# int-brain-lab/mtscomp

Hardware: AMD Instinct MI355X
Metric: compress + decompress GB/s (raw int16) (higher is better)
Workload: dtype int16

## Files before the change

### mtscomp_amd/csrc/inflate.hip

```cpp
#include <stdlib.h>

#include <vector>

#include "common.h"

namespace mts {

struct BitIn {
    const u32 *w;
    u64 nwords;
    u64 widx;
    u64 buf;
    u32 cnt;
    u32 nextw;
    u64 pos;
    u64 end;
    const u32 *lw = nullptr;
    u64 lw0 = 0;
    u32 lwn = 0;
    __device__ __forceinline__ void init(const u8 *base, u64 byte_off, u64 byte_len, u64 start_bit)
    {
        const u64 a = (u64)(base + byte_off);
        w = (const u32 *)(a & ~(u64)3);
        const u64 bit0 = (a & 3) * 8;
// ... 675 lines not shown
            if (o2 < 12) t0 |= (u64)k << (5 * o2); else t1 |= (u64)k << (5 * (o2 - 12));
        }
    }
    s.t0 = t0; s.t1 = t1;
    s.nlen = nlen; s.total = nlen + ndist;
    s.idx = 0; s.prev = 0; s.len256 = 0; s.maxl = 0; s.maxd = 0; s.kl = 0; s.kd = 0;
    return true;
}

__device__ __forceinline__ int vh_step(VhState &s)
{
    BitIn &br = s.br;
    br.refill();
    const u32 pk = br.peek();
    const u32 v7 = __brev(pk) >> 25, vb = __builtin_amdgcn_perm(v7, v7, 0u) | 0x80808080u;
    const u32 nge = (u32)__popc((vb - s.lima) & 0x80808080u) + (u32)__popc((vb - s.limb) & 0x80808080u);
    const u32 clen = 1 + nge;
    const int si = (int)(((u32)(s.so64 >> (8 * nge)) & 0xffu) + ((v7 - ((u32)(s.lo64 >> (8 * nge)) & 0xffu)) >> (6 - nge)));
    const int sym = (int)((si < 12 ? s.t0 >> (5 * si) : s.t1 >> (5 * (si - 12))) & 31);
    const u32 t4 = 4u * (u32)(max(sym, 15) - 15);
    const u32 xb = (0x7320u >> t4) & 15u;
    const int rep = (int)(((0xb331u >> t4) & 15u) + __builtin_amdgcn_ubfe(pk, clen, xb));
    br.skip(clen + xb);
    const int idx = s.idx, nlen = s.nlen;
    const int val = sym < 16 ? sym : sym == 16 ? s.prev : 0;
    if (sym >= 16 && ((sym == 16 && idx == 0) || idx + rep > s.total)) return -1;
    s.prev = val;
    if (val) {
        const int nl = idx >= nlen ? 0 : (idx + rep <= nlen ? rep : nlen - idx);
        const int nd = rep - nl;
        s.kl += (u32)nl << (15 - val);
        s.kd += (u32)nd << (15 - val);
        if (nl && val > s.maxl) s.maxl = val;
        if (nd && val > s.maxd) s.maxd = val;
        if (idx <= 256 && 256 < idx + rep) s.len256 = val;
        if (s.kl > 32768u || s.kd > 32768u) return -1;
    }
    s.idx = idx + rep;
    if (br.pos > br.end) return -1;
    if (s.idx < s.total) return 0;
    if (s.len256 == 0) return -1;
    if (s.kl > 32768u || (s.kl < 32768u && s.maxl != 1)) return -1;
    if (s.kd > 32768u || (s.kd < 32768u && s.maxd > 1)) return -1;
    return 1;
}

struct InfFast {
    u64 cand_off;
    u32 cand_cap;
    u32 true_off;
    u32 true_cap;
    u32 pad;
};
struct CandRes {
    u64 end_bit;
    u32 ntok, nout, nsub;
    u32 ok;
    u32 bfinal;
    u32 rows;
};
struct TrueBlk {
    u64 start_bit;
    u32 cand;
    u32 tok_off;
    u32 ntok;
    u32 chunk;
};
constexpr int PASSA_STAGE_WORDS = 64 * 1024 / 32 + 16;
#ifndef MTS_PASSB_STAGE_WORDS
#define MTS_PASSB_STAGE_WORDS 2304
#endif
constexpr int PASSB_STAGE_WORDS = MTS_PASSB_STAGE_WORDS;
constexpr int SUBCAP = 512;
constexpr u32 SUB_BITS = 1024;
#ifndef MTS_SUB_TARGET
#define MTS_SUB_TARGET 1024
#endif
constexpr u32 SUB_TARGET = MTS_SUB_TARGET;
constexpr u32 SUB_MIN = 256;
#ifndef MTS_INF_ROWCAP
#define MTS_INF_ROWCAP 192
#endif
constexpr u32 ROWCAP = MTS_INF_ROWCAP;
constexpr int ROUNDS_MAX = (SUBCAP + 63) / 64;
static inline u64 rows_rounds_of(u64 c_len) { return c_len * 8 / (64 * 640) + 32; }

#ifndef MTS_SCAN_SPANS
#define MTS_SCAN_SPANS 1
#endif
#ifndef MTS_PA_LEAN
#define MTS_PA_LEAN 1
#endif
constexpr int SCAN_SPANS = MTS_SCAN_SPANS;
constexpr u64 SCAN_FINAL_ZONE_BITS = 8ull * 256 * 1024;
constexpr int SCAN_L1_CAP = 14336;

__global__ __launch_bounds__(SCAN_THREADS) void k_inf_scan(const u8 *__restrict__ cdata, const InfChunk *__restrict__ chunks,
                                                           const InfFast *__restrict__ fast, u64 *__restrict__ cand_pos,
                                                           u32 *__restrict__ cand_cnt, u64 *__restrict__ surv_list,
                                                           u32 *__restrict__ surv_cnt, u32 surv_cap, u64 final_zone_bits)
{
    const int ci = blockIdx.y;
    const InfChunk ch = chunks[ci];
    if (ch.c_len < 8) return;
    const u64 a = (u64)(cdata + ch.c_off);
    const u32 *w = (const u32 *)(a & ~(u64)3);
    const u64 bit0 = (a & 3) * 8, end = bit0 + 8 * ch.c_len, nwords = (end + 31) >> 5;
    if ((u64)blockIdx.x * SCAN_SPANS * SCAN_SPAN_BITS >= end) return;
    __shared__ u32 sw[SCAN_THREADS + SCAN_TAIL];
    __shared__ u16 l1[SCAN_L1_CAP];
    __shared__ u32 surv[SCAN_SURV_CAP];
    __shared__ u32 wsum[16];
    __shared__ u32 nsurv;
    __shared__ u8 ktab[4096];
    const int tid = threadIdx.x, wave = tid >> 6, lane = tid & 63;
    for (int i = tid; i < 4096; i += SCAN_THREADS) {
        u32 k = 0;
        for (int f = 0; f < 4; f++) k += (0x80u >> ((i >> (3 * f)) & 7)) & 0x7f;
        ktab[i] = (u8)(k < 255 ? k : 255);
    }
    __shared__ u32 gbase_s;
    for (int sp = 0; sp < SCAN_SPANS; sp++) {
    const u64 span0 = ((u64)blockIdx.x * SCAN_SPANS + sp) * SCAN_SPAN_BITS;
    if (span0 >= end) break;
    const u64 word0 = span0 >> 5;
    __syncthreads();
    for (int i = tid; i < SCAN_THREADS + SCAN_TAIL; i += SCAN_THREADS) sw[i] = word0 + i < nwords ? w[word0 + i] : 0;
    if (tid == 0) nsurv = 0;
    __syncthreads();
    const u32 w0 = sw[tid], w1 = sw[tid + 1];
#define S_(j) __builtin_amdgcn_alignbit(w1, w0, j)
    u32 m = ~S_(1) & S_(2);
    m &= ~(S_(4) & S_(5) & S_(6) & S_(7));
    m &= ~(S_(9) & S_(10) & S_(11) & S_(12));
#undef S_
    if (span0 + SCAN_SPAN_BITS + final_zone_bits <= end) m &= ~w0;
    {
        const u64 o0 = span0 + (u64)tid * 32;
        const u64 first_ok = bit0 + 16;
        if (o0 + 32 <= first_ok || o0 + 100 > end) {
            u32 keep = 0;
            for (int k = 0; k < 32; k++) if (o0 + k >= first_ok && o0 + k + 100 <= end) keep |= 1u << k;
            m &= keep;
        } else if (o0 < first_ok) m &= ~0u << (u32)(first_ok - o0);
    }
    const u32 cntm = __popc(m);
    const u32 incl = wave_incl_scan_dpp(cntm), ex = incl - cntm;
    if (lane == 63) wsum[wave] = incl;
    __syncthreads();
    u32 base = 0, n1 = 0;
    for (int q = 0; q < 16; q++) { if (q < wave) base += wsum[q]; n1 += wsum[q]; }
    n1 = n1 < (u32)SCAN_L1_CAP ? n1 : (u32)SCAN_L1_CAP;
    {
        u32 slot = base + ex, mm = m;
        while (mm) {
            const int k = __ffs(mm) - 1;
            mm &= mm - 1;
            if (slot < (u32)SCAN_L1_CAP) l1[slot] = (u16)(tid * 32 + k);
            slot++;
        }
    }
    __syncthreads();
    for (u32 it = tid; it < n1; it += SCAN_THREADS) {
        const u32 rel = l1[it];
        const u32 wi = rel >> 5, k = rel & 31;
        const u32 x0 = sw[wi], x1 = sw[wi + 1], x2 = sw[wi + 2], x3 = sw[wi + 3];
// ... 71 lines not shown
                    }
                    active = vh_setup(s, w, nwords, end, o, row, VAL_STAGE);
                }
            }
            if (!__any(active)) {
                if (base + cnt >= stop) break;
                continue;
            }
        }
        for (int k = 0; k < VAL_STEPS; k++) {
            if (active) {
                const int r = vh_step(s);
                if (r) {
                    active = false;
                    if (r > 0) {
                        const InfFast f = fast[ci];
                        const u32 slot = atomicAdd(&cand_cnt[ci], 1u);
                        if (slot < f.cand_cap) cand_pos[f.cand_off + slot] = o;
                    }
                }
            }
        }
    }
}

__global__ __launch_bounds__(256) void k_inf_sortc(const InfFast *__restrict__ fast, u64 *__restrict__ cand_pos,
                                                   u64 *__restrict__ cand_tmp, u32 *__restrict__ cand_cnt)
{
    const int ci = blockIdx.x;
    const InfFast f = fast[ci];
    const u32 n = min(cand_cnt[ci], f.cand_cap);
    u64 *p = cand_pos + f.cand_off, *t = cand_tmp + f.cand_off;
    for (u32 i = threadIdx.x; i < n; i += 256) t[i] = p[i];
    __syncthreads();
    for (u32 i = threadIdx.x; i < n; i += 256) {
        const u64 v = t[i];
        u32 r = 0;
        for (u32 j = 0; j < n; j++) r += t[j] < v;
        p[r] = v;
    }
}

enum { SPAN_CONT = 0, SPAN_EOB = 1, SPAN_ERR = 2 };

template <int MODE>
__device__ __forceinline__ void decode_span(BitIn &br, LaneLds &L, const u32 *lutl, const u32 *lutd, u64 stop, u32 &ntok, u32 &nout,
                                            int &flag, u32 *tk, u32 want)
{
    flag = SPAN_CONT;
    ntok = 0; nout = 0;
    for (;;) {
        if (MODE == 2) { if (ntok >= want) break; }
        else if (br.pos >= stop) break;
        u32 tok, olen;
        const int t = decode_token_lut(br, L, lutl, lutd, tok, olen);
        if (t < 0 || br.pos > br.end) { flag = SPAN_ERR; break; }
        if (t == 1) { flag = SPAN_EOB; break; }
        const u32 np = lz_pieces(tok, olen);
        if (MODE == 2) lz_emit_pieces(tk + ntok, tok, olen);
        ntok += np; nout += olen;
    }
}

template <int MODE>
__device__ __forceinline__ void decode_span_fast(BitL &br, LaneLds &L, const u32 *lutl, const u32 *lutd, u32 stop, u32 end, u32 &ntok,
                                                 u32 &nout, int &flag, u32 *tk, u32 want)
{
    flag = SPAN_CONT;
    ntok = 0; nout = 0;
    for (;;) {
        if (MODE == 2) { if (ntok >= want) break; }
        else if (br.pos >= stop) break;
        u32 tok, olen;
        const int t = decode_token_lut(br, L, lutl, lutd, tok, olen);
        if (t < 0 || br.pos > end) { flag = SPAN_ERR; break; }
        if (t == 1) { flag = SPAN_EOB; break; }
        const u32 np = lz_pieces(tok, olen);
        if (MODE == 2) lz_emit_pieces(tk + ntok, tok, olen);
        ntok += np; nout += olen;
    }
}

__device__ __forceinline__ void decode_span_rows(BitL &br, LaneLds &L, const u32 *lutl, const u32 *lutd, u32 stop, u32 end, u32 &ntok,
                                                 u32 &nout, int &flag, u32 *row, u32 cap, bool &ovf)
{
    flag = SPAN_CONT;
    ntok = 0; nout = 0; ovf = false;
    for (;;) {
        if (br.pos >= stop) break;
        u32 tok, olen;
        const int t = decode_token_lut(br, L, lutl, lutd, tok, olen);
        if (t < 0 || br.pos > end) { flag = SPAN_ERR; break; }
        if (t == 1) { flag = SPAN_EOB; break; }
        const u32 np = lz_pieces(tok, olen);
        if (ntok + np <= cap) lz_emit_pieces(row + ntok, tok, olen);
        else ovf = true;
        ntok += np; nout += olen;
    }
}

__device__ __forceinline__ void decode_span_exit_w(BitW &br, LaneLds &L, const u32 *lutl, const u32 *lutd, u32 stop, u32 end, int &flag)
{
    flag = SPAN_CONT;
    for (;;) {
        if (br.pos >= stop) break;
        u32 tok, olen;
        const int t = decode_token_w(br, L, lutl, lutd, tok, olen);
        if (t < 0 || br.pos > end) { flag = SPAN_ERR; break; }
        if (t == 1) { flag = SPAN_EOB; break; }
    }
}
__device__ __forceinline__ void decode_span_rows_w(BitW &br, LaneLds &L, const u32 *lutl, const u32 *lutd, u32 stop, u32 end, u32 &ntok,
                                                   u32 &nout, int &flag, u32 *row, u32 cap, bool &ovf)
{
    flag = SPAN_CONT;
    ntok = 0; nout = 0; ovf = false;
    for (;;) {
        if (br.pos >= stop) break;
        u32 tok, olen;
        const int t = decode_token_w(br, L, lutl, lutd, tok, olen);
        if (t < 0 || br.pos > end) { flag = SPAN_ERR; break; }
        if (t == 1) { flag = SPAN_EOB; break; }
        const u32 np = lz_pieces(tok, olen);
        if (ntok + np <= cap) lz_emit_pieces(row + ntok, tok, olen);
        else ovf = true;
        ntok += np; nout += olen;
    }
}

__device__ __forceinline__ int first_lane(u64 m) { return m ? __ffsll((long long)m) - 1 : 64; }

__global__ __launch_bounds__(64) void k_inf_passA(const u8 *__restrict__ cdata, const InfChunk *__restrict__ chunks,
                                                  const InfFast *__restrict__ fast, const u32 *__restrict__ slot_chunk,
                                                  const u64 *__restrict__ cand_pos, const u32 *__restrict__ cand_cnt,
                                                  CandRes *__restrict__ cres, uint2 *__restrict__ subs, u32 *__restrict__ rows,
                                                  u32 *__restrict__ row_ctr, u32 rounds_cap, u32 *__restrict__ round_row)
{
    const u32 slot = blockIdx.x;
    const u32 ci = slot_chunk[slot];
    const InfFast f = fast[ci];
    const u32 k = slot - (u32)f.cand_off;
    if (k >= min(cand_cnt[ci], f.cand_cap)) return;
    const InfChunk ch = chunks[ci];
    __shared__ __attribute__((aligned(16))) u8 tabs[INF_SET_BYTES];
    LaneLds L;
    L.bind(tabs, 1, 0);
    const int lane = threadIdx.x;
    BitIn br;
    br.init(cdata, ch.c_off, ch.c_len, 0);
    const u64 o = cand_pos[slot];
    __shared__ u32 stage[PASSA_STAGE_WORDS];
    stage_stream_words(stage, br, o >> 5, SCAN_TAIL + 8, (u32)threadIdx.x, 64);
    __builtin_amdgcn_wave_barrier();
    br.lw = stage; br.lw0 = o >> 5; br.lwn = SCAN_TAIL + 8;
    br.seek(o);
    CandRes r;
    r.end_bit = 0; r.ntok = 0; r.nout = 0; r.nsub = 0; r.ok = 0; r.bfinal = 0; r.rows = 0;
    const u32 hdr = br.get(3);
    r.bfinal = hdr & 1;
    __shared__ u32 lut_s[LUT_BYTES / 4];
    u32 *lutl = lut_s, *lutd = lut_s + (1 << LUT_LBITS);
    u32 *LC = lutd + (1 << LUT_DBITS), *DC = LC + 16;
    static_assert(SCAN_TAIL + 8 + PARSE_WAVE_WORDS <= PASSA_STAGE_WORDS, "the header's words and the parse's scratch fit the stage");
    const int rc = parse_tables_wave(br, L, hdr >> 1, LC, DC, stage + SCAN_TAIL + 8, lane);
    if (rc != INF_OK) { if (lane == 0) cres[slot] = r; return; }
    __builtin_amdgcn_wave_barrier();
    build_luts(L, lutl, lutd, lane);
    __builtin_amdgcn_wave_barrier();
    uint2 *sub = subs + (u64)slot * SUBCAP;
    u32 sub_bits = SUB_BITS;
    {
        const u32 ncand_c = min(cand_cnt[ci], f.cand_cap);
        const u64 next_o = k + 1 < ncand_c ? cand_pos[slot + 1] : 8ull * ch.c_len;
        const u64 est = next_o > br.pos ? next_o - br.pos : 0;
        const u64 rounds = (est + 64ull * SUB_TARGET - 1) / (64ull * SUB_TARGET);
        if (rounds >= 1 && rounds * 64 + 64 <= (u64)SUBCAP - 1) {
            const u64 per = (est + 64 * rounds - 1) / (64 * rounds);
            sub_bits = (u32)((per + 31) & ~31ull);
            sub_bits = sub_bits < SUB_MIN ? SUB_MIN : sub_bits > SUB_BITS ? SUB_BITS : sub_bits;
        }
    }
    const u64 base0 = br.pos;
    u64 base = base0;
    u32 tot_tok = 0, tot_out = 0, nsub = 0;
    bool done = false, fail = false, rows_ok = true;
    br.lw = nullptr; br.lwn = 0;
#if MTS_PA_LEAN
    BitW bl;
#else
    BitL bl;
#endif
    bl.w = stage;
    while (!done && !fail) {
        const u64 wb0 = base >> 5;
        const u32 bofs = (u32)(base & 31);
        __builtin_amdgcn_wave_barrier();
        const u32 stage_words = 64 * sub_bits / 32 + 16;
        stage_stream_words(stage, br, wb0, stage_words, (u32)lane, 64);
        __builtin_amdgcn_wave_barrier();
        const u64 end_rel64 = br.end - (wb0 << 5);
        const u32 end_rel = end_rel64 < 0x7fffffffull ? (u32)end_rel64 : 0x7fffffffu;
        const u32 stop = bofs + (u32)(lane + 1) * sub_bits;
        u32 start = bofs + (u32)lane * sub_bits, ex;
        u32 nt, no; int fl;
        u32 rb = 0;
        if (lane == 0) rb = atomicAdd(row_ctr, 1u);
        rb = (u32)__builtin_amdgcn_readfirstlane((int)rb);
        const bool have_rows = rb < rounds_cap;
        u32 *row = rows + ((u64)(have_rows ? rb : 0) * 64 + lane) * ROWCAP;
        bool ovf = false;
        bl.seek(start);
#if MTS_PA_LEAN
        decode_span_exit_w(bl, L, lutl, lutd, stop, end_rel, fl);
#else
        decode_span_fast<0>(bl, L, lutl, lutd, stop, end_rel, nt, no, fl, nullptr, 0);
#endif
        ex = bl.pos;
        bool counted = false;
        for (int it = 0; it < 66; it++) {
            const u32 pex = __shfl_up(ex, 1, 64);
            const u32 want_start = lane == 0 ? bofs : pex;
            const u64 stopm = __ballot(fl != SPAN_CONT);
            const int fstop = first_lane(stopm);
            const bool valid = lane <= fstop;
            const bool redo = valid && (!counted || want_start != start);
            if (!__any(redo)) break;
            if (redo) {
                start = want_start;
                bl.seek(start);
#if MTS_PA_LEAN
                decode_span_rows_w(bl, L, lutl, lutd, stop, end_rel, nt, no, fl, row, have_rows ? ROWCAP : 0u, ovf);
#else
                decode_span_rows(bl, L, lutl, lutd, stop, end_rel, nt, no, fl, row, have_rows ? ROWCAP : 0u, ovf);
#endif
                ex = bl.pos;
                counted = true;
            }
        }
        const u64 stopm = __ballot(fl != SPAN_CONT);
        const int fstop = first_lane(stopm);
        const bool valid = lane <= fstop && counted;
        const u32 pex = __shfl_up(ex, 1, 64);
        const bool bad = valid && lane > 0 && pex != start;
        if (__any(bad) || __any(lane <= fstop && !counted)) { fail = true; break; }
        u32 x = valid ? nt : 0, y = valid ? no : 0;
#pragma unroll
        for (int off = 1; off < 64; off <<= 1) {
            const u32 xx = __shfl_up(x, off, 64), yy = __shfl_up(y, off, 64);
            if (lane >= off) { x += xx; y += yy; }
        }
        const int nvalid = fstop < 64 ? fstop + 1 : 64;
        if (nsub + nvalid > SUBCAP - 1) {
            if (sub_bits < SUB_BITS) { sub_bits = SUB_BITS; base = base0; tot_tok = 0; tot_out = 0; nsub = 0; rows_ok = true; continue; }
            fail = true; break;
        }
        if (!have_rows || __any(valid && ovf)) rows_ok = false;
        if (lane == 0) round_row[(u64)slot * ROUNDS_MAX + (nsub >> 6)] = rb;
        if (valid) sub[nsub + lane] = make_uint2((u32)((wb0 << 5) + start - o), tot_tok + x - nt);
        const u32 rt = __shfl(x, nvalid - 1, 64), ro = __shfl(y, nvalid - 1, 64);
        tot_tok += rt; tot_out += ro;
        nsub += nvalid;
        if (fstop < 64) {
            const int ffl = __shfl(fl, fstop, 64);
            const u32 fex = __shfl(ex, fstop, 64);
            if (ffl == SPAN_EOB) { done = true; r.end_bit = (wb0 << 5) + fex; }
            else fail = true;
        } else base = (wb0 << 5) + (u32)__shfl(ex, 63, 64);
    }
    if (lane == 0) {
        if (done && !fail) {
            sub[nsub] = make_uint2(0, tot_tok);
            r.ok = 1; r.ntok = tot_tok; r.nout = tot_out; r.nsub = nsub; r.rows = rows_ok ? 1u : 0u;
        }
        cres[slot] = r;
    }
}

constexpr int CHAIN_NEED_SEQ = 1;
constexpr u64 CHAIN_INLINE_BYTES = 4096;
constexpr int CHAIN_LDS_CAND = 1024;

__global__ __launch_bounds__(64) void k_inf_chain(const u8 *__restrict__ cdata, const InfChunk *__restrict__ chunks,
                                                  const InfFast *__restrict__ fast, const u64 *__restrict__ cand_pos,
                                                  const u32 *__restrict__ cand_cnt, const CandRes *__restrict__ cres,
                                                  TrueBlk *__restrict__ tblk, u32 *__restrict__ true_cnt,
                                                  InfResult *__restrict__ res, int *__restrict__ seq_flag)
{
    const int ci = blockIdx.x;
    const InfChunk ch = chunks[ci];
    const InfFast f = fast[ci];
    const int lane = threadIdx.x;
    __shared__ __attribute__((aligned(16))) u8 tabs[INF_SET_BYTES];
    InfResult r;
    r.status = MTS_CHUNK_OK; r.n_out = 0; r.ntok = 0; r.adler_stored = 0; r.end_bit = 0;
    const u8 *cb = cdata + ch.c_off;
    bool ok = ch.c_len >= 2;
    if (ok) {
        const u32 cmf = cb[0], flg = cb[1];
        ok = ((cmf << 8) | flg) % 31 == 0 && (cmf & 15) == 8 && (cmf >> 4) <= 7 && !(flg & 0x20);
    }
    if (!ok) { if (lane == 0) { r.status = MTS_CHUNK_CORRUPT; res[ci] = r; seq_flag[ci] = 0; true_cnt[ci] = 0; } return; }
    BitIn br;
    br.init(cdata, ch.c_off, ch.c_len, 16);
    const u32 ncand = min(cand_cnt[ci], f.cand_cap);
    const bool cand_overflow = cand_cnt[ci] > f.cand_cap;
    const u64 *cp = cand_pos + f.cand_off;
    u32 cur = 0;
    u64 pos = br.pos;
    u32 ntok = 0, ntrue = 0;
    u64 nout = 0;
    bool last = false, need_seq = cand_overflow, enough = false;
    LaneLds L;
    L.bind(tabs, 1, 0);
    {
        __shared__ uint4 c_rec[CHAIN_LDS_CAND];
        __shared__ u64 c_pos[CHAIN_LDS_CAND];
        __shared__ u16 c_succ[CHAIN_LDS_CAND];
        if (ncand <= (u32)CHAIN_LDS_CAND && ncand > 0 && !need_seq) {
            for (u32 i = lane; i < ncand; i += 64) {
                const CandRes c = cres[f.cand_off + i];
                c_pos[i] = cp[i];
                c_rec[i] = make_uint4((u32)c.end_bit, (u32)(c.end_bit >> 32), c.ntok, (c.nout & 0x3fffffffu) | (c.ok ? 1u << 30 : 0u) | (c.bfinal ? 1u << 31 : 0u));
            }
            __builtin_amdgcn_wave_barrier();
            auto find = [&](u64 p) -> u32 {
                u32 lo = 0, hi = ncand;
                while (lo < hi) { const u32 mid = (lo + hi) >> 1; if (c_pos[mid] < p) lo = mid + 1; else hi = mid; }
                return (lo < ncand && c_pos[lo] == p) ? lo : 0xffffu;
            };
            for (u32 i = lane; i < ncand; i += 64) {
                const uint4 e = c_rec[i];
                c_succ[i] = (u16)(((e.w >> 30) & 1) ? find((u64)e.x | ((u64)e.y << 32)) : 0xffffu);
            }
            __builtin_amdgcn_wave_barrier();
            u32 i = find(pos);
            while (i != 0xffffu) {
                const uint4 e = c_rec[i];
                if (!((e.w >> 30) & 1)) break;
                const u32 b_ntok = e.z, b_nout = e.w & 0x3fffffffu;
                if (ntrue >= f.true_cap || (u64)ntok + b_ntok > (u64)ch.n_expect + 1 || nout + b_nout > ch.n_expect) { need_seq = true; break; }
// ... 17 lines not shown
    bool have = false;
    u64 hv = ~0ull, h_end = 0;
    u32 h_ntok = 0, h_nout = 0, h_ok = 0, h_bfinal = 0;
    while (!last && !need_seq && !enough) {
        int found = -1, fl = 0;
        for (;;) {
            if (!have) {
                hb = cur;
                const u32 i = hb + lane;
                hv = i < ncand ? cp[i] : ~0ull;
                h_ok = 0;
                if (i < ncand) { const CandRes c = cres[f.cand_off + i]; h_end = c.end_bit; h_ntok = c.ntok; h_nout = c.nout; h_ok = c.ok; h_bfinal = c.bfinal; }
                have = true;
            }
            const u64 ge = __ballot(hv >= pos);
            if (ge == 0) { cur = hb + 64; have = false; if (cur >= ncand) break; continue; }
            fl = first_lane(ge);
            const u64 fv = (u64)(u32)__builtin_amdgcn_readlane((int)(u32)hv, fl) | ((u64)(u32)__builtin_amdgcn_readlane((int)(u32)(hv >> 32), fl) << 32);
            cur = hb + (u32)fl;
            if (fv == pos) found = (int)cur;
            break;
        }
        u32 b_ntok = 0, b_nout = 0, b_cand = 0xffffffffu;
        u64 b_end = 0;
        bool b_ok = false;
        auto rl = [&](u32 x) -> u32 { return (u32)__builtin_amdgcn_readlane((int)x, fl); };
        if (found >= 0 && rl(h_ok)) {
            b_ok = true; b_ntok = rl(h_ntok); b_nout = rl(h_nout); b_end = (u64)rl((u32)h_end) | ((u64)rl((u32)(h_end >> 32)) << 32);
            b_cand = (u32)(f.cand_off + found); last = rl(h_bfinal);
        }
        if (!b_ok) {
            br.seek(pos);
            const u32 hdr = br.get(3);
            if ((hdr >> 1) == 0 && br.pos <= br.end) {
                br.seek((br.pos + 7) & ~7ull);
                const u32 len = br.get(16), nlen = br.get(16);
                if (br.pos > br.end || (len ^ 0xffff) != nlen || br.pos + 8ull * len > br.end) { need_seq = true; break; }
                b_ntok = len; b_nout = len; b_end = br.pos + 8ull * len; last = hdr & 1;
            } else {
                br.seek(pos);
                u32 nt = 0; u64 no = nout; bool lst = false;
                const int st = decode_block<false>(br, L, nullptr, nt, no, nout + CHAIN_INLINE_BYTES, lst);
                if (st != INF_OK) { need_seq = true; break; }
                b_ntok = nt; b_nout = (u32)(no - nout); b_end = br.pos; last = lst;
            }
        }
        if (ntrue >= f.true_cap || (u64)ntok + b_ntok > (u64)ch.n_expect + 1 || nout + b_nout > ch.n_expect) { need_seq = true; break; }
        if (lane == 0) {
            TrueBlk tb;
            tb.start_bit = pos; tb.cand = b_cand; tb.tok_off = ntok; tb.ntok = b_ntok; tb.chunk = (u32)ci;
            tblk[f.true_off + ntrue] = tb;
        }
        ntrue++;
        ntok += b_ntok; nout += b_nout;
        pos = b_end;
        if (ch.n_need && nout >= ch.n_need) enough = true;
    }
    if (enough) {
        r.end_bit = pos; r.n_out = (u32)nout; r.ntok = ntok;
    } else if (need_seq && ch.n_need) {
        r.status = MTS_CHUNK_NEEDMORE;
        need_seq = false;
        ntrue = 0;
    } else if (!need_seq) {
        const u64 tb = (pos + 7) & ~7ull;
        if (tb + 32 > br.end) r.status = MTS_CHUNK_CORRUPT;
        else {
            const u8 *t = (const u8 *)br.w + (tb >> 3);
            r.adler_stored = ((u32)t[0] << 24) | ((u32)t[1] << 16) | ((u32)t[2] << 8) | t[3];
            r.end_bit = tb + 32;
            if (nout != ch.n_expect) r.status = MTS_CHUNK_BADSIZE;
        }
        r.n_out = (u32)nout; r.ntok = ntok;
    } else {
        r.end_bit = pos; r.n_out = (u32)nout; r.ntok = ntok;
    }
    if (lane == 0) {
        res[ci] = r;
        seq_flag[ci] = need_seq ? CHAIN_NEED_SEQ : 0;
        true_cnt[ci] = ntrue;
    }
}

constexpr int MOVE_THREADS = 256;
__global__ __launch_bounds__(MOVE_THREADS) void k_inf_move_rows(const InfChunk *__restrict__ chunks, const InfFast *__restrict__ fast,
                                                                const u32 *__restrict__ tslot_chunk, const TrueBlk *__restrict__ tblk,
                                                                const u32 *__restrict__ true_cnt, const CandRes *__restrict__ cres,
                                                                const uint2 *__restrict__ subs, const u32 *__restrict__ rows,
                                                                const u32 *__restrict__ round_row, u32 *__restrict__ tokens)
{
    const u32 slot = blockIdx.x;
    const u32 ci = tslot_chunk[slot];
    const InfFast f = fast[ci];
    if (slot - f.true_off >= true_cnt[ci]) return;
    const TrueBlk tb = tblk[slot];
    if (tb.cand == 0xffffffffu || !cres[tb.cand].rows) return;
    __shared__ u32 ys[SUBCAP + 1], rid[SUBCAP];
    const u32 nsub = cres[tb.cand].nsub, total = tb.ntok;
    const uint2 *sub = subs + (u64)tb.cand * SUBCAP;
    for (u32 j = threadIdx.x; j < nsub; j += MOVE_THREADS) {
        ys[j] = sub[j].y;
        rid[j] = round_row[(u64)tb.cand * ROUNDS_MAX + (j >> 6)] * 64 + (j & 63);
    }
    if (threadIdx.x == 0) ys[nsub] = 0xffffffffu;
    __syncthreads();
    u32 *tk = tokens + chunks[ci].tok_off + tb.tok_off;
    constexpr u32 U = 16;
    u32 jw = 0;
    for (u32 t0 = 0; t0 < total; t0 += U * MOVE_THREADS) {
        while (ys[jw + 1] <= t0) jw++;
        u32 v[U], j = jw;
#pragma unroll
        for (u32 u = 0; u < U; u++) {
            const u32 t = min(t0 + u * MOVE_THREADS + threadIdx.x, total - 1);
            while (ys[j + 1] <= t) j++;
            v[u] = rows[(u64)rid[j] * ROWCAP + (t - ys[j])];
        }
#pragma unroll
        for (u32 u = 0; u < U; u++) {
            const u32 t = t0 + u * MOVE_THREADS + threadIdx.x;
            if (t < total) tk[t] = v[u];
        }
    }
}

#ifndef MTS_PASSB_WAVES
#define MTS_PASSB_WAVES 1
#endif
constexpr int PASSB_WAVES = MTS_PASSB_WAVES;
__global__ __launch_bounds__(64 * PASSB_WAVES) void k_inf_passB(const u8 *__restrict__ cdata, const InfChunk *__restrict__ chunks,
                                                  const InfFast *__restrict__ fast, const u32 *__restrict__ tslot_chunk,
                                                  const TrueBlk *__restrict__ tblk, const u32 *__restrict__ true_cnt,
                                                  const CandRes *__restrict__ cres, const uint2 *__restrict__ subs,
                                                  u32 *__restrict__ tokens, InfResult *__restrict__ res, int use_rows)
{
    const u32 slot = blockIdx.x;
    const u32 ci = tslot_chunk[slot];
    const InfFast f = fast[ci];
    if (slot - f.true_off >= true_cnt[ci]) return;
    const TrueBlk tb = tblk[slot];
    const InfChunk ch = chunks[ci];
    __shared__ __attribute__((aligned(16))) u8 tabs[INF_SET_BYTES];
    LaneLds L;
    L.bind(tabs, 1, 0);
    const int lane = threadIdx.x & 63, wave = threadIdx.x >> 6;
    BitIn br;
    br.init(cdata, ch.c_off, ch.c_len, 0);
    br.seek(tb.start_bit);
    u32 *tk = tokens + ch.tok_off + tb.tok_off;
    if (tb.cand == 0xffffffffu) {
        if (wave) return;
        const u32 hdr0 = br.get(3);
        if ((hdr0 >> 1) == 0) {
            br.seek((br.pos + 7) & ~7ull);
            const u32 len = br.get(16);
            const u8 *src = (const u8 *)br.w + ((br.pos + 16) >> 3);
            if (len != tb.ntok) { if (lane == 0) res[ci].status = MTS_CHUNK_CORRUPT; return; }
            for (u32 i = lane; i < len; i += 64) tk[i] = src[i];
            return;
        }
        br.seek(tb.start_bit);
        u32 nt = 0; u64 no = 1ull << 40; bool lst;
        if (lane == 0) {
            const int st = decode_block<true>(br, L, tk, nt, no, ~0ull, lst);
            if (st != INF_OK || nt != tb.ntok) res[ci].status = MTS_CHUNK_CORRUPT;
        }
        return;
    }
    __shared__ u32 stage_s[PASSB_WAVES][PASSB_STAGE_WORDS];
    if (use_rows && cres[tb.cand].rows) return;
    const u32 hdr = br.get(3);
    __shared__ u32 lut_s[LUT_BYTES / 4];
    u32 *lutl = lut_s, *lutd = lut_s + (1 << LUT_LBITS);
    u32 *LC = lutd + (1 << LUT_DBITS), *DC = LC + 16;
    __shared__ int hdr_rc;
    if (wave == 0) {
        const int rc = parse_tables(br, L, hdr >> 1, LC, DC);
        if (lane == 0) hdr_rc = rc;
        __builtin_amdgcn_wave_barrier();
        if (rc == INF_OK) build_luts(L, lutl, lutd, lane);
    }
    __syncthreads();
    if (hdr_rc != INF_OK) { if (threadIdx.x == 0) res[ci].status = MTS_CHUNK_CORRUPT; return; }
    const u32 nsub = cres[tb.cand].nsub;
    const uint2 *sub = subs + (u64)tb.cand * SUBCAP;
    u32 *stage = stage_s[wave];
    for (u32 j0 = 64 * (u32)wave; j0 < nsub; j0 += 64 * PASSB_WAVES) {
        const u32 j = j0 + lane;
        const u32 jl = min(j0 + 64, nsub);
        const u64 round_end = jl < nsub ? tb.start_bit + sub[jl].x : cres[tb.cand].end_bit;
        const u64 wlo = (tb.start_bit + sub[j0].x) >> 5, whi = (round_end >> 5) + 3;
        __builtin_amdgcn_wave_barrier();
        const bool staged = whi - wlo < (u64)PASSB_STAGE_WORDS;
        if (staged) {
            const u32 nw = (u32)(whi - wlo) + 1;
            stage_stream_words(stage, br, wlo, nw, (u32)lane, 64);
        }
        __builtin_amdgcn_wave_barrier();
        if (j < nsub) {
            const uint2 a = sub[j], b = sub[j + 1];
            u32 nt, no; int fl;
            if (staged) {
                BitL bl;
                bl.w = stage;
// ... 1004 lines not shown
        sa += s1; sb += (nn - p) * (u64)s1 - s2;
    } else {
        for (u32 q = p; q < r.n_out; q++) {
            const u32 c = cells[q];
            const u32 kq = seg_of(q);
            const u8 v = (u8)(c < 256 ? c : W[(size_t)kq * LZ_WIN + ((b0s[kq] + c - 256) & (LZ_WIN - 1))]);
            out[q] = v;
            sa += v; sb += (nn - q) * (u64)v;
        }
    }
    }
    finish();
}

__global__ __launch_bounds__(64) void k_inf_finish(const InfChunk *__restrict__ chunks, InfResult *__restrict__ res,
                                                   const u64 *__restrict__ adler_acc, int n_chunks, int *__restrict__ status_out,
                                                   const u64 *__restrict__ seg_adler)
{
    const int ci = blockIdx.x * 64 + threadIdx.x;
    if (ci >= n_chunks) return;
    InfResult r = res[ci];
    if (r.status == MTS_CHUNK_OK && chunks[ci].n_need == 0) {
        u64 fa = 0, fb = 0;
        if (seg_adler) for (int k = 0; k < LZ_MAXSEG * LZ_FLUSHERS; k++) { fa += seg_adler[((size_t)ci * LZ_MAXSEG * LZ_FLUSHERS + k) * 2]; fb += seg_adler[((size_t)ci * LZ_MAXSEG * LZ_FLUSHERS + k) * 2 + 1]; }
        const u32 a = (u32)((1 + adler_acc[2 * ci] + fa) % 65521u), b = (u32)((chunks[ci].n_expect + adler_acc[2 * ci + 1] + fb) % 65521u);
        if (((b << 16) | a) != r.adler_stored) r.status = MTS_CHUNK_CORRUPT;
    }
    res[ci].status = r.status;
    status_out[ci] = r.status;
}

__global__ __launch_bounds__(256) void k_inf_fill_slots(const InfFast *__restrict__ fast, u32 *__restrict__ slot_chunk, u32 *__restrict__ tslot_chunk)
{
    const InfFast f = fast[blockIdx.x];
    for (u32 k = threadIdx.x; k < f.cand_cap; k += 256) slot_chunk[f.cand_off + k] = blockIdx.x;
    for (u32 k = threadIdx.x; k < f.true_cap; k += 256) tslot_chunk[f.true_off + k] = blockIdx.x;
}

static inline u32 cand_cap_of(u64 c_len) { return (u32)(c_len / 4096 + 64); }

struct InfLayout {
    size_t so, nn, fast, cand_cnt, true_cnt, seq_flag, slot_chunk, tslot_chunk, cand_pos, cand_tmp, cres, tblk, subs, gb_off, gbase, tb_off, tile_base, surv, surv_cnt, plan, win, sym, rows,
        round_row, row_ctr, gflag, seg_adler, end;
    u32 total_cand, total_true, surv_cap, rounds_cap;
    int nseg;
};
static InfLayout inf_layout(int n_chunks, const u64 *c_lens, const u32 *n_expect)
{
    InfLayout l;
    u64 tc = 0;
    for (int i = 0; i < n_chunks; i++) tc += cand_cap_of(c_lens[i]);
    l.total_cand = (u32)tc;
    l.total_true = (u32)(2 * tc);
    size_t o = 0;
    auto take = [&](size_t bytes) { const size_t r = o; o += align_up(bytes, 256); return r; };
    l.so = take(8 * (size_t)n_chunks); l.nn = take(4 * (size_t)n_chunks); l.fast = take(sizeof(InfFast) * (size_t)n_chunks);
    l.gb_off = take(8 * (size_t)n_chunks); l.tb_off = take(8 * (size_t)n_chunks);
    l.cand_cnt = take(4 * (size_t)n_chunks); l.true_cnt = take(4 * (size_t)n_chunks); l.seq_flag = take(4 * (size_t)n_chunks);
    l.slot_chunk = take(4 * (size_t)l.total_cand); l.tslot_chunk = take(4 * (size_t)l.total_true);
    l.cand_pos = take(8 * (size_t)l.total_cand); l.cand_tmp = take(8 * (size_t)l.total_cand);
    l.cres = take(sizeof(CandRes) * (size_t)l.total_cand); l.tblk = take(sizeof(TrueBlk) * (size_t)l.total_true);
    l.subs = take(sizeof(uint2) * (size_t)SUBCAP * l.total_cand);
    size_t ng = 0;
    for (int i = 0; i < n_chunks; i++) ng += ((size_t)n_expect[i] + 2 + 63) / 64 + 2;
    l.gbase = take(4 * ng);
    l.tile_base = take(4 * (ng / GS_TILE + 2 * (size_t)n_chunks + 16));
    u64 cbits = 0;
    for (int i = 0; i < n_chunks; i++) cbits += 8 * c_lens[i];
    l.surv_cap = (u32)(cbits / 256 + 65536);
    l.surv = take(8 * (size_t)l.surv_cap);
    l.surv_cnt = take(256);
    l.nseg = 1;
    if (n_chunks < 128) { l.nseg = 256 / n_chunks; if (l.nseg > LZ_MAXSEG) l.nseg = LZ_MAXSEG; }
    if (const char *e = getenv("MTS_LZ_SEGS")) { l.nseg = atoi(e); if (l.nseg < 1) l.nseg = 1; if (l.nseg > LZ_MAXSEG) l.nseg = LZ_MAXSEG; }
    l.plan = take(sizeof(LzPlan) * (size_t)n_chunks);
    l.win = take(l.nseg > 1 ? (size_t)n_chunks * LZ_MAXSEG * LZ_WIN : 0);
    size_t cells = 0;
    for (int i = 0; i < n_chunks; i++) cells += align_up((u64)n_expect[i] + STREAM_PAD, STREAM_ALIGN);
    u64 rounds = 0;
    for (int i = 0; i < n_chunks; i++) rounds += rows_rounds_of(c_lens[i]);
    if (const char *e = getenv("MTS_INF_ROW_ROUNDS")) rounds = (u64)atoll(e);
    if (rounds > 0x3ffffffull) rounds = 0x3ffffffull;
    l.rounds_cap = (u32)rounds;
    const size_t row_bytes = (size_t)rounds * 64 * ROWCAP * 4 + 256, sym_bytes = l.nseg > 1 ? 2 * cells + 4096 : 0;
    l.sym = take(row_bytes > sym_bytes ? row_bytes : sym_bytes);
    l.rows = l.sym;
    l.round_row = take(4 * (size_t)ROUNDS_MAX * l.total_cand);
    l.row_ctr = take(256);
    l.gflag = take(l.nseg > 1 ? cells / LZ_FLUSH + (size_t)n_chunks + 64 : 0);
    l.seg_adler = take(l.nseg > 1 ? (size_t)n_chunks * LZ_MAXSEG * LZ_FLUSHERS * 16 : 0);
    l.end = o;
    return l;
}

size_t inflate_scratch_bytes(int n_chunks, const u64 *c_lens, const u32 *n_expect) { return inf_layout(n_chunks, c_lens, n_expect).end + 256; }

static void dbg_status(hipStream_t st, const InfResult *d_res, int n_chunks, const char *where)
{
    if (!getenv("MTS_DEBUG_STATUS")) return;
    std::vector<InfResult> h(n_chunks);
    (void)hipStreamSynchronize(st);
    (void)hipMemcpy(h.data(), d_res, sizeof(InfResult) * n_chunks, hipMemcpyDeviceToHost);
    fprintf(stderr, "[status %s]", where);
    for (int i = 0; i < n_chunks; i++) fprintf(stderr, " %d:(st %d nout %u ntok %u)", i, h[i].status, h[i].n_out, h[i].ntok);
    fprintf(stderr, "\n");
}

int launch_inflate(hipStream_t st, const u8 *d_cdata, const InfChunk *d_chunks, const InfChunk *h_chunks, int n_chunks,
                   u8 *d_stream, u32 *d_tokens, InfResult *d_res, u64 *d_adler_acc, u32 max_n, int *d_status_out,
                   void *d_scratch, void *engine)
{
    if (n_chunks == 0) return MTS_OK;
    MTS_LDS_ATTR(k_inf_lz, LZ_LDS);
    MTS_LDS_ATTR(k_inf_lz_seg, LZ2_LDS);
    std::vector<u64> lens(n_chunks), so(n_chunks);
    std::vector<u32> nn(n_chunks);
    u64 max_clen = 0;
    for (int i = 0; i < n_chunks; i++) {
        lens[i] = h_chunks[i].c_len; so[i] = h_chunks[i].stream_off; nn[i] = h_chunks[i].n_expect;
        if (lens[i] > max_clen) max_clen = lens[i];
    }
    const InfLayout l = inf_layout(n_chunks, lens.data(), nn.data());
    if (getenv("MTS_DEBUG_STATUS"))
        for (int i = 0; i < n_chunks; i++) {
            std::vector<u8> hb(h_chunks[i].c_len);
            (void)hipStreamSynchronize(st);
            (void)hipMemcpy(hb.data(), d_cdata + h_chunks[i].c_off, hb.size(), hipMemcpyDeviceToHost);
            u32 a = 1, b2 = 0;
            for (u8 v : hb) { a = (a + v) % 65521u; b2 = (b2 + a) % 65521u; }
            fprintf(stderr, "[chunk %d] device copy of the compressed bytes: adler32 %08x\n", i, (b2 << 16) | a);
        }
    if (getenv("MTS_DEBUG_STATUS"))
        for (int i = 0; i < n_chunks; i++)
            fprintf(stderr, "[chunk %d] c_off %llu c_len %llu n_expect %u n_need %u stream_off %llu tok_off %llu\n", i, (unsigned long long)h_chunks[i].c_off,
                    (unsigned long long)h_chunks[i].c_len, h_chunks[i].n_expect, h_chunks[i].n_need, (unsigned long long)h_chunks[i].stream_off, (unsigned long long)h_chunks[i].tok_off);
    u8 *S = (u8 *)d_scratch;
    const size_t hst_bytes = l.cand_cnt - l.so;
    u8 *hst = inflate_host_stage(engine, hst_bytes);
    u64 *h_so = (u64 *)(hst + (l.so - l.so)), *h_gb = (u64 *)(hst + (l.gb_off - l.so)), *h_tb = (u64 *)(hst + (l.tb_off - l.so));
    u32 *h_nn = (u32 *)(hst + (l.nn - l.so));
    InfFast *h_fast = (InfFast *)(hst + (l.fast - l.so));
    {
        u64 a = 0, b2 = 0, co = 0;
        u32 to = 0;
        for (int i = 0; i < n_chunks; i++) {
            const u64 ng1 = ((u64)nn[i] + 2 + 63) / 64 + 2;
            h_gb[i] = a; a += ng1;
            h_tb[i] = b2; b2 += ng1 / GS_TILE + 2;
            h_so[i] = so[i]; h_nn[i] = nn[i];
            h_fast[i].cand_off = co; h_fast[i].cand_cap = cand_cap_of(lens[i]);
            h_fast[i].true_off = to; h_fast[i].true_cap = 2 * h_fast[i].cand_cap; h_fast[i].pad = 0;
            co += h_fast[i].cand_cap; to += h_fast[i].true_cap;
        }
    }
    MTS_HIP(hipMemcpyAsync(S + l.so, hst, hst_bytes, hipMemcpyHostToDevice, st));
    MTS_HIP(hipMemsetAsync(S + l.cand_cnt, 0, 4 * (size_t)n_chunks, st));
    hipLaunchKernelGGL(k_inf_fill_slots, dim3(n_chunks), dim3(256), 0, st, (const InfFast *)(S + l.fast), (u32 *)(S + l.slot_chunk), (u32 *)(S + l.tslot_chunk));
    const InfFast *d_fast = (const InfFast *)(S + l.fast);
    u64 *d_cand_pos = (u64 *)(S + l.cand_pos), *d_cand_tmp = (u64 *)(S + l.cand_tmp);
    u32 *d_cand_cnt = (u32 *)(S + l.cand_cnt), *d_true_cnt = (u32 *)(S + l.true_cnt);
    int *d_seq = (int *)(S + l.seq_flag);
    CandRes *d_cres = (CandRes *)(S + l.cres);
    TrueBlk *d_tblk = (TrueBlk *)(S + l.tblk);
    uint2 *d_subs = (uint2 *)(S + l.subs);
    const bool fast_path = getenv("MTS_INFLATE_SEQ") == nullptr;
    int lz_workers = LZ_WORKERS;
    if (const char *e = getenv("MTS_LZ_WORKERS")) { lz_workers = atoi(e); if (lz_workers < 1) lz_workers = 1; if (lz_workers > LZ_WORKERS) lz_workers = LZ_WORKERS; }
// ... 106 lines not shown
```

Measured before the change: 35.59.

## Store raw tokens column-major in per-round slabs and expand them in move kernel

```diff
diff --git a/mtscomp_amd/csrc/inflate.hip b/mtscomp_amd/csrc/inflate.hip
--- a/mtscomp_amd/csrc/inflate.hip
+++ b/mtscomp_amd/csrc/inflate.hip
@@ -781,6 +781,7 @@
 #define MTS_INF_ROWCAP 192
 #endif
 constexpr u32 ROWCAP = MTS_INF_ROWCAP;
+constexpr u32 SLAB_WORDS = (ROWCAP + 1) * 64;
 constexpr int ROUNDS_MAX = (SUBCAP + 63) / 64;
 static inline u64 rows_rounds_of(u64 c_len) { return c_len * 8 / (64 * 640) + 32; }
 
@@ -1018,20 +1019,19 @@
 }
 
 __device__ __forceinline__ void decode_span_rows(BitL &br, LaneLds &L, const u32 *lutl, const u32 *lutd, u32 stop, u32 end, u32 &ntok,
-                                                 u32 &nout, int &flag, u32 *row, u32 cap, bool &ovf)
+                                                 u32 &nout, int &flag, u32 *col, u32 cap, u32 &nsym, bool &ovf)
 {
     flag = SPAN_CONT;
-    ntok = 0; nout = 0; ovf = false;
+    ntok = 0; nout = 0; nsym = 0; ovf = false;
     for (;;) {
         if (br.pos >= stop) break;
         u32 tok, olen;
         const int t = decode_token_lut(br, L, lutl, lutd, tok, olen);
         if (t < 0 || br.pos > end) { flag = SPAN_ERR; break; }
         if (t == 1) { flag = SPAN_EOB; break; }
-        const u32 np = lz_pieces(tok, olen);
-        if (ntok + np <= cap) lz_emit_pieces(row + ntok, tok, olen);
+        if (nsym < cap) col[nsym * 64] = tok;
         else ovf = true;
-        ntok += np; nout += olen;
+        nsym++; ntok += lz_pieces(tok, olen); nout += olen;
     }
 }
 
@@ -1047,20 +1047,19 @@
     }
 }
 __device__ __forceinline__ void decode_span_rows_w(BitW &br, LaneLds &L, const u32 *lutl, const u32 *lutd, u32 stop, u32 end, u32 &ntok,
-                                                   u32 &nout, int &flag, u32 *row, u32 cap, bool &ovf)
+                                                   u32 &nout, int &flag, u32 *col, u32 cap, u32 &nsym, bool &ovf)
 {
     flag = SPAN_CONT;
-    ntok = 0; nout = 0; ovf = false;
+    ntok = 0; nout = 0; nsym = 0; ovf = false;
     for (;;) {
         if (br.pos >= stop) break;
         u32 tok, olen;
         const int t = decode_token_w(br, L, lutl, lutd, tok, olen);
         if (t < 0 || br.pos > end) { flag = SPAN_ERR; break; }
         if (t == 1) { flag = SPAN_EOB; break; }
-        const u32 np = lz_pieces(tok, olen);
-        if (ntok + np <= cap) lz_emit_pieces(row + ntok, tok, olen);
+        if (nsym < cap) col[nsym * 64] = tok;
         else ovf = true;
-        ntok += np; nout += olen;
+        nsym++; ntok += lz_pieces(tok, olen); nout += olen;
     }
 }
 
@@ -1143,7 +1142,8 @@
         if (lane == 0) rb = atomicAdd(row_ctr, 1u);
         rb = (u32)__builtin_amdgcn_readfirstlane((int)rb);
         const bool have_rows = rb < rounds_cap;
-        u32 *row = rows + ((u64)(have_rows ? rb : 0) * 64 + lane) * ROWCAP;
+        u32 *slab = rows + (u64)(have_rows ? rb : 0) * SLAB_WORDS;
+        u32 nsym = 0;
         bool ovf = false;
         bl.seek(start);
 #if MTS_PA_LEAN
@@ -1165,9 +1165,9 @@
                 start = want_start;
                 bl.seek(start);
 #if MTS_PA_LEAN
-                decode_span_rows_w(bl, L, lutl, lutd, stop, end_rel, nt, no, fl, row, have_rows ? ROWCAP : 0u, ovf);
+                decode_span_rows_w(bl, L, lutl, lutd, stop, end_rel, nt, no, fl, slab + 64 + lane, have_rows ? ROWCAP : 0u, nsym, ovf);
 #else
-                decode_span_rows(bl, L, lutl, lutd, stop, end_rel, nt, no, fl, row, have_rows ? ROWCAP : 0u, ovf);
+                decode_span_rows(bl, L, lutl, lutd, stop, end_rel, nt, no, fl, slab + 64 + lane, have_rows ? ROWCAP : 0u, nsym, ovf);
 #endif
                 ex = bl.pos;
                 counted = true;
@@ -1192,6 +1192,7 @@
         }
         if (!have_rows || __any(valid && ovf)) rows_ok = false;
         if (lane == 0) round_row[(u64)slot * ROUNDS_MAX + (nsub >> 6)] = rb;
+        if (have_rows) slab[lane] = valid ? nsym : 0u;
         if (valid) sub[nsub + lane] = make_uint2((u32)((wb0 << 5) + start - o), tot_tok + x - nt);
         const u32 rt = __shfl(x, nvalid - 1, 64), ro = __shfl(y, nvalid - 1, 64);
         tot_tok += rt; tot_out += ro;
@@ -1375,7 +1376,19 @@
     }
 }
 
-constexpr int MOVE_THREADS = 256;
+#ifndef MTS_MOVE_WAVES
+#define MTS_MOVE_WAVES 2
+#endif
+#ifndef MTS_MOVE_KT
+#define MTS_MOVE_KT 32
+#endif
+#ifndef MTS_MOVE_W
+#define MTS_MOVE_W 64
+#endif
+constexpr int MOVE_WAVES = MTS_MOVE_WAVES;
+constexpr u32 MOVE_KT = MTS_MOVE_KT, MOVE_W = MTS_MOVE_W, MOVE_PITCH = MOVE_W + 1;
+static_assert(MOVE_W >= 33 && MOVE_W <= 64, "a lane's stage holds the 33 pieces of the longest copy; a wave writes a stage row with one store");
+constexpr int MOVE_THREADS = 64 * MOVE_WAVES;
 __global__ __launch_bounds__(MOVE_THREADS) void k_inf_move_rows(const InfChunk *__restrict__ chunks, const InfFast *__restrict__ fast,
                                                                 const u32 *__restrict__ tslot_chunk, const TrueBlk *__restrict__ tblk,
                                                                 const u32 *__restrict__ true_cnt, const CandRes *__restrict__ cres,
@@ -1388,31 +1401,64 @@
     if (slot - f.true_off >= true_cnt[ci]) return;
     const TrueBlk tb = tblk[slot];
     if (tb.cand == 0xffffffffu || !cres[tb.cand].rows) return;
-    __shared__ u32 ys[SUBCAP + 1], rid[SUBCAP];
-    const u32 nsub = cres[tb.cand].nsub, total = tb.ntok;
+    __shared__ u32 tile_s[MOVE_WAVES][MOVE_KT * 64], stage_s[MOVE_WAVES][64 * MOVE_PITCH];
+    const u32 lane = threadIdx.x & 63, wave = threadIdx.x >> 6;
+    u32 *tile = tile_s[wave], *stg = stage_s[wave] + lane * MOVE_PITCH;
+    const u32 *stage = stage_s[wave];
+    const u32 nsub = cres[tb.cand].nsub;
     const uint2 *sub = subs + (u64)tb.cand * SUBCAP;
-    for (u32 j = threadIdx.x; j < nsub; j += MOVE_THREADS) {
-        ys[j] = sub[j].y;
-        rid[j] = round_row[(u64)tb.cand * ROUNDS_MAX + (j >> 6)] * 64 + (j & 63);
-    }
-    if (threadIdx.x == 0) ys[nsub] = 0xffffffffu;
-    __syncthreads();
     u32 *tk = tokens + chunks[ci].tok_off + tb.tok_off;
-    constexpr u32 U = 16;
-    u32 jw = 0;
-    for (u32 t0 = 0; t0 < total; t0 += U * MOVE_THREADS) {
-        while (ys[jw + 1] <= t0) jw++;
-        u32 v[U], j = jw;
-#pragma unroll
-        for (u32 u = 0; u < U; u++) {
-            const u32 t = min(t0 + u * MOVE_THREADS + threadIdx.x, total - 1);
-            while (ys[j + 1] <= t) j++;
-            v[u] = rows[(u64)rid[j] * ROWCAP + (t - ys[j])];
-        }
-#pragma unroll
-        for (u32 u = 0; u < U; u++) {
-            const u32 t = t0 + u * MOVE_THREADS + threadIdx.x;
-            if (t < total) tk[t] = v[u];
+    for (u32 j0 = 64 * wave; j0 < nsub; j0 += 64 * MOVE_WAVES) {
+        const u32 nrows = min(64u, nsub - j0);
+        const u32 *slab = rows + (u64)round_row[(u64)tb.cand * ROUNDS_MAX + (j0 >> 6)] * SLAB_WORDS;
+        u32 cnt = lane < nrows ? min(slab[lane], ROWCAP) : 0u;
+        u32 dst = lane < nrows ? sub[j0 + lane].y : 0u;
+        const u32 lim = lane < nrows ? sub[j0 + lane + 1].y : 0u;
+        u32 depth = cnt, k = 0;
+#pragma unroll
+        for (int off = 1; off < 64; off <<= 1) depth = max(depth, (u32)__shfl_xor((int)depth, off, 64));
+        depth = (u32)__builtin_amdgcn_readfirstlane((int)depth);
+        for (u32 k0 = 0; k0 < depth; k0 += MOVE_KT) {
+            const u32 kt = min(MOVE_KT, depth - k0);
+            __builtin_amdgcn_wave_barrier();
+            {
+                u32 v[MOVE_KT];
+#pragma unroll
+                for (u32 i = 0; i < MOVE_KT; i++) v[i] = i < kt ? slab[(1 + k0 + i) * 64 + lane] : 0u;
+#pragma unroll
+                for (u32 i = 0; i < MOVE_KT; i++) tile[i * 64 + lane] = v[i];
+            }
+            __builtin_amdgcn_wave_barrier();
+            const u32 kend = min(cnt, k0 + kt);
+            while (__any(k < kend)) {
+                u32 n = 0;
+                u32 nxt = tile[min(k - k0, MOVE_KT - 1) * 64 + lane];
+                while (k < kend) {
+                    const u32 tok = nxt;
+                    const u32 olen = (tok >> 31) ? ((tok >> 16) & 0xff) + 3 : 1u;
+                    const u32 np = lz_pieces(tok, olen);
+                    if (n + np > MOVE_W) break;
+                    if (dst + n + np > lim) { cnt = 0; k = kend; break; }
+                    k++;
+                    nxt = tile[min(k - k0, MOVE_KT - 1) * 64 + lane];
+                    lz_emit_pieces(stg + n, tok, olen);
+                    n += np;
+                }
+                __builtin_amdgcn_wave_barrier();
+                for (u32 j = 0; j < nrows; j += 8) {
+                    u32 v[8];
+#pragma unroll
+                    for (u32 u = 0; u < 8; u++) v[u] = stage[(j + u) * MOVE_PITCH + lane];
+#pragma unroll
+                    for (u32 u = 0; u < 8; u++) {
+                        const u32 nj = (u32)__builtin_amdgcn_readlane((int)n, (int)(j + u));
+                        const u32 dj = (u32)__builtin_amdgcn_readlane((int)dst, (int)(j + u));
+                        if (lane < nj) tk[dj + lane] = v[u];
+                    }
+                }
+                dst += n;
+                __builtin_amdgcn_wave_barrier();
+            }
         }
     }
 }
@@ -2583,7 +2629,7 @@
     if (const char *e = getenv("MTS_INF_ROW_ROUNDS")) rounds = (u64)atoll(e);
     if (rounds > 0x3ffffffull) rounds = 0x3ffffffull;
     l.rounds_cap = (u32)rounds;
-    const size_t row_bytes = (size_t)rounds * 64 * ROWCAP * 4 + 256, sym_bytes = l.nseg > 1 ? 2 * cells + 4096 : 0;
+    const size_t row_bytes = (size_t)rounds * SLAB_WORDS * 4 + 256, sym_bytes = l.nseg > 1 ? 2 * cells + 4096 : 0;
     l.sym = take(row_bytes > sym_bytes ? row_bytes : sym_bytes);
     l.rows = l.sym;
     l.round_row = take(4 * (size_t)ROUNDS_MAX * l.total_cand);
```

Result: slower. 34.61 (-2.8%).
